# XikunLiu-huskit/GLIO

Hardware: NVIDIA B200
Metric: sliding-window FGO iterations/sec (20 KF, 100k surf pts/scan) (higher is better)
Workload: dtype f64

## Files before the change

### glio_b200/api.py

```python
import ctypes as C
import os

import numpy as np

_HERE = os.path.dirname(os.path.abspath(__file__))
_LIB_PATH = os.path.join(_HERE, "libglio_b200.so")
_LIB = None

HOST, DEVICE = 0, 1
MATCH_VALID, MATCH_FAIL_RADIUS, MATCH_FAIL_PLANE, MATCH_FAIL_WEIGHT = 0, 1, 2, 3


class GlioError(RuntimeError):
    pass


class Params(C.Structure):
    _fields_ = [("kd_max_radius", C.c_double), ("surf_dist_thres", C.c_double), ("lidar_const", C.c_double),
                ("weight_min", C.c_double), ("huber_delta", C.c_double), ("q_lb", C.c_double * 4),
                ("t_lb", C.c_double * 3), ("batch_max_radius", C.c_double), ("batch_dist_thres", C.c_double),
                ("batch_score", C.c_double), ("cell_size", C.c_float), ("keep_debug", C.c_int32), ("unit_score", C.c_int32)]


def lib():
    global _LIB
    if _LIB is None:
        if not os.path.exists(_LIB_PATH):
            raise GlioError(f"{_LIB_PATH} not found: build it with `python -c 'import __graft_entry__ as g; g.build()'` "
                            "(glio_b200 has no CPU fallback)")
        L = C.CDLL(_LIB_PATH)
        L.glio_last_error.restype = C.c_char_p
        L.glio_last_error.argtypes = [C.c_void_p]
        L.glio_stream.restype = C.c_void_p
        L.glio_stream.argtypes = [C.c_void_p]
        L.glio_launch_count.restype = C.c_int64
        L.glio_launch_count.argtypes = [C.c_void_p]
        L.glio_destroy.argtypes = [C.c_void_p]
        L.glio_destroy.restype = None
        L.glio_marg_prior_destroy.argtypes = [C.c_void_p]
        L.glio_marg_prior_destroy.restype = None
        L.glio_marg_prior_create.restype = C.c_void_p
        _LIB = L
    return _LIB


def default_params(**kw):
    p = Params()
    lib().glio_default_params(C.byref(p))
    for k, v in kw.items():
        if k in ("q_lb", "t_lb"):
            arr = getattr(p, k)
            for i, x in enumerate(v):
                arr[i] = float(x)
        else:
            setattr(p, k, v)
    return p


def _ptr(a):
    if a is None:
        return None
    if isinstance(a, np.ndarray):
        return a.ctypes.data_as(C.c_void_p)
    if isinstance(a, int):
        return C.c_void_p(a)
    raise TypeError(type(a))


def _points_arg(xyz):
    if isinstance(xyz, np.ndarray):
        a = np.ascontiguousarray(xyz, dtype=np.float32)
        if a.ndim == 1:
            a = a.reshape(-1, 3)
        return a, _ptr(a), a.shape[0], a.shape[1], HOST
    if hasattr(xyz, "data_ptr"):
        assert xyz.is_cuda and xyz.is_contiguous() and xyz.dtype.itemsize == 4
        return xyz, C.c_void_p(xyz.data_ptr()), xyz.shape[0], xyz.shape[1], DEVICE
    raise TypeError("points must be a numpy array or a CUDA torch tensor")


class Context:
    def __init__(self, device=0, params=None, **kw):
        self._lib = lib()
        self.params = params if params is not None else default_params(**kw)
        self._h = C.c_void_p()
        rc = self._lib.glio_create(C.c_int(device), C.byref(self.params), C.byref(self._h))
        if rc != 0:
            msg = self._lib.glio_last_error(None)
            raise GlioError(f"glio_create failed ({rc}): {msg.decode() if msg else ''}")
        self._keep = []

    def close(self):
        if getattr(self, "_h", None):
            self._lib.glio_destroy(self._h)
            self._h = None

    def __del__(self):
        try:
            self.close()
        except Exception:
            pass

    def _chk(self, rc):
        if rc != 0:
            msg = self._lib.glio_last_error(self._h)
            raise GlioError(f"glio error {rc}: {msg.decode() if msg else ''}")

    @property
    def stream(self):
        return self._lib.glio_stream(self._h)

    @property
    def launch_count(self):
        return int(self._lib.glio_launch_count(self._h))

    def synchronize(self):
        self._chk(self._lib.glio_synchronize(self._h))

    def lidar_pose(self, pose_body):
        pb = np.ascontiguousarray(pose_body, np.float64)
        t2 = np.zeros(3); q2 = np.zeros(4)
        self._lib.glio_lidar_pose(C.byref(self.params), _ptr(pb), _ptr(t2), _ptr(q2))
        return t2, q2

    KERNELS = ["k_feat_curvature", "k_feat_select", "k_feat_voxel", "k_feat_offsets", "k_feat_gather", "k_knn_tile", "k_knn_tile2", "k_defer_scatter", "k_knn_box_start", "k_knn_grow", "k_knn_box_far", "k_knn_far", "k_knn_box_cells", "k_knn_team", "k_make_pairs", "k_knn_search", "k_knn_deferred", "k_knn_thread", "k_knn_box", "k_plane_fit", "k_plane_fit_pair", "k_eval_unary", "k_eval_unary_cost", "k_transform_hist", "k_order_scatter",
               "k_compact", "k_flags", "k_cell_hist", "k_cell_scatter", "k_load_bounds", "k_scan_block", "k_scan_add",
               "k_eval_binary", "k_eval_binary_cost", "k_bin_assemble",
               "k_lm_transform", "k_vox_hist", "k_vox_scatter", "k_vox_sort", "k_vox_flags", "k_vox_centroid", "k_init_bounds"]

    def lib_profile(self, on):
        self._chk(self._lib.glio_profile_enable(self._h, C.c_int(1 if on else 0)))

    def lib_profile_read(self):
        out = {}
        for k in self.KERNELS:
            ms = C.c_double(0); n = C.c_int64(0)
            self._chk(self._lib.glio_profile_get(self._h, k.encode(), C.byref(ms), C.byref(n)))
            if n.value:
                out[k] = (ms.value, int(n.value))
        return out

    def knn_fallback_queries(self, reset=False):
        n = C.c_int64(0)
        self._chk(self._lib.glio_get_stats(self._h, C.byref(n), C.c_int(1 if reset else 0)))
        return int(n.value)

    def get_match_counts(self, W, active=True):
        nm = np.zeros(W, np.int64); na = np.zeros(W, np.int64)
        self._chk(self._lib.glio_get_match_counts(self._h, C.c_int(W), _ptr(nm), _ptr(na)))
        return na if active else nm

    def set_map(self, xyz):
        keep, p, n, stride, mem = _points_arg(xyz)
        self._map_keep = keep
        self._chk(self._lib.glio_set_map(self._h, p, C.c_int64(n), C.c_int(stride), C.c_int(mem)))

    def map_prefetch(self, xyz):
        keep, p, n, stride, mem = _points_arg(xyz)
        assert mem == HOST
        self._map_pf_keep = keep
        self._chk(self._lib.glio_map_prefetch(self._h, p, C.c_int64(n), C.c_int(stride)))

    def localmap_clear(self):
        self._chk(self._lib.glio_localmap_clear(self._h))

    def localmap_push(self, cloud_xyz, t, q, at_front=False):
        keep, p, n, stride, mem = _points_arg(cloud_xyz)
        t = np.ascontiguousarray(t, np.float64); q = np.ascontiguousarray(q, np.float64)
        self._chk(self._lib.glio_localmap_push(self._h, C.c_int(1 if at_front else 0), p, C.c_int64(n), C.c_int(stride), C.c_int(mem), _ptr(t), _ptr(q)))

    def localmap_pop_front(self):
        self._chk(self._lib.glio_localmap_pop_front(self._h))

    def localmap_size(self):
        nf = C.c_int(0); npnt = C.c_int64(0)
        self._chk(self._lib.glio_localmap_size(self._h, C.byref(nf), C.byref(npnt)))
        return nf.value, int(npnt.value)

    def localmap_build(self, leaf=0.4):
        n = C.c_int64(0)
        self._chk(self._lib.glio_localmap_build(self._h, C.c_float(leaf), C.byref(n)))
        return int(n.value)

    def get_map(self):
        n = C.c_int64(0)
        self._chk(self._lib.glio_get_map(self._h, C.c_int64(0), None, C.byref(n)))
        out = np.empty((int(n.value), 3), np.float32)
        self._chk(self._lib.glio_get_map(self._h, C.c_int64(len(out)), _ptr(out), C.byref(n)))
        return out

    def assoc_scan_to_map(self, slot, scan_xyz, t, q):
        keep, p, n, stride, mem = _points_arg(scan_xyz)
        self._keep.append(keep); self._keep = self._keep[-64:]
        t = np.ascontiguousarray(t, np.float64); q = np.ascontiguousarray(q, np.float64)
        nm = C.c_int64(0)
        self._chk(self._lib.glio_assoc_scan_to_map(self._h, C.c_int(slot), p, C.c_int64(n), C.c_int(stride), C.c_int(mem),
                                                   _ptr(t), _ptr(q), C.byref(nm)))
        return int(nm.value)

    def window_set_scans(self, scans):
        args = [_points_arg(s) for s in scans]
        self._scan_keep = [a[0] for a in args]
        W = len(args)
        ptrs = (C.c_void_p * W)(*[a[1] for a in args])
        Q = (C.c_int64 * W)(*[a[2] for a in args])
        strides = {a[3] for a in args}; mems = {a[4] for a in args}
        assert len(strides) == 1 and len(mems) == 1
        self._chk(self._lib.glio_window_set_scans(self._h, C.c_int(W), ptrs, Q, C.c_int(strides.pop()), C.c_int(mems.pop())))

    def window_set_scan(self, slot, scan):
        keep, p, n, stride, mem = _points_arg(scan)
        if not hasattr(self, "_slot_keep"):
            self._slot_keep = {}
        self._slot_keep[slot] = keep
        self._chk(self._lib.glio_window_set_scan(self._h, C.c_int(slot), p, C.c_int64(n), C.c_int(stride), C.c_int(mem)))

    def window_slide(self, W):
        self._chk(self._lib.glio_window_slide(self._h, C.c_int(W)))

    def window_associate(self, poses_body):
        pb = np.ascontiguousarray(poses_body, np.float64).reshape(-1, 7)
        W = len(pb)
        nm = np.zeros(W, np.int64)
        self._chk(self._lib.glio_window_associate(self._h, C.c_int(W), _ptr(pb), _ptr(nm)))
        return nm

    def get_matches(self, slot, capacity):
        cp = np.empty((capacity, 3), np.float32); nsd = np.empty((capacity, 4), np.float32)
        w = np.empty(capacity, np.float32); src = np.empty(capacity, np.int32)
        n = C.c_int64(0)
        self._chk(self._lib.glio_get_matches(self._h, C.c_int(slot), C.c_int64(capacity), _ptr(cp), _ptr(nsd), _ptr(w), _ptr(src), C.byref(n)))
        n = int(n.value)
        return dict(cp=cp[:n], nsd=nsd[:n], weight=w[:n], src=src[:n], n=n)

    def get_assoc_debug(self, slot, Q):
        out = dict(status=np.empty(Q, np.uint8), idx5=np.empty((Q, 5), np.int32), sqd5=np.empty((Q, 5), np.float32),
                   pm=np.empty((Q, 3), np.float32), plane=np.empty((Q, 4), np.float64))
        self._chk(self._lib.glio_get_assoc_debug(self._h, C.c_int(slot), C.c_int64(Q), _ptr(out["status"]), _ptr(out["idx5"]),
                                                 _ptr(out["sqd5"]), _ptr(out["pm"]), _ptr(out["plane"])))
        return out

    def select(self, slot, keep):
        if keep is None:
            self._chk(self._lib.glio_select(self._h, C.c_int(slot), None, C.c_int64(-1)))
            return
        k = np.ascontiguousarray(keep, np.int32)
        self._chk(self._lib.glio_select(self._h, C.c_int(slot), _ptr(k), C.c_int64(len(k))))

    def eval_unary(self, poses_body, jac_kind=0, want_jac=True):
        pb = np.ascontiguousarray(poses_body, np.float64).reshape(-1, 7)
        W = len(pb)
        H = np.zeros((W, 6, 6)) if want_jac else None
        g = np.zeros((W, 6)) if want_jac else None
        cost = np.zeros(W)
        self._chk(self._lib.glio_eval_unary(self._h, C.c_int(W), _ptr(pb), C.c_int(jac_kind), _ptr(H), _ptr(g), _ptr(cost)))
        return dict(H=H, g=g, cost=cost)

    def eval_unary_residuals(self, slot, pose_body, capacity, jac_kind=0):
        pb = np.ascontiguousarray(pose_body, np.float64)
        r = np.empty(capacity); J = np.empty((capacity, 6)); n = C.c_int64(0)
        self._chk(self._lib.glio_eval_unary_residuals(self._h, C.c_int(slot), _ptr(pb), C.c_int(jac_kind), C.c_int64(capacity),
                                                      _ptr(r), _ptr(J), C.byref(n)))
        n = int(n.value)
        return r[:n], J[:n]


class SolverOptions(C.Structure):
    _fields_ = [("max_num_iterations", C.c_int32), ("dogleg_type", C.c_int32), ("use_nonmonotonic_steps", C.c_int32),
                ("max_consecutive_nonmonotonic_steps", C.c_int32), ("initial_trust_region_radius", C.c_double),
                ("max_trust_region_radius", C.c_double), ("min_trust_region_radius", C.c_double),
                ("min_relative_decrease", C.c_double), ("min_lm_diagonal", C.c_double), ("max_lm_diagonal", C.c_double),
                ("max_num_consecutive_invalid_steps", C.c_int32), ("jacobi_scaling", C.c_int32),
                ("function_tolerance", C.c_double), ("gradient_tolerance", C.c_double), ("parameter_tolerance", C.c_double),
                ("fuse_candidate_jacobian", C.c_int32), ("trust_region_strategy", C.c_int32)]


class Iteration(C.Structure):
    _fields_ = [("iteration", C.c_int32), ("step_is_valid", C.c_int32), ("step_is_successful", C.c_int32), ("reserved", C.c_int32),
                ("cost", C.c_double), ("cost_change", C.c_double), ("gradient_max_norm", C.c_double), ("gradient_norm", C.c_double),
# ... 340 lines not shown
```

### glio_b200/csrc/assoc.cu

```cuda
#include "common.cuh"
#include "devmath.cuh"
#include "knn_common.cuh"

namespace glio {

__device__ __forceinline__ int find_seg(const SegDesc* __restrict__ segs, int nseg, int64_t g) {
  int lo = 0, hi = nseg - 1;
  while (lo < hi) {
    int mid = (lo + hi + 1) >> 1;
    if (segs[mid].offset <= g) lo = mid; else hi = mid - 1;
  }
  return lo;
}

__global__ void __launch_bounds__(256) k_transform_hist(GridDesc grid, const SegDesc* __restrict__ segs, int nseg,
                                                        int64_t Qt, float4* __restrict__ pm, uint16_t* __restrict__ segid,
                                                        int* __restrict__ cell_count) {
  const int64_t g = (int64_t)blockIdx.x * blockDim.x + threadIdx.x;
  if (g >= Qt) return;
  const int s = find_seg(segs, nseg, g);
  const SegDesc& sd = segs[s];
  const float* src = sd.src + (g - sd.offset) * sd.stride;
  float p[3] = {src[0], src[1], src[2]};
  PoseD P;
  P.t[0] = sd.t[0]; P.t[1] = sd.t[1]; P.t[2] = sd.t[2];
  P.q[0] = sd.q[0]; P.q[1] = sd.q[1]; P.q[2] = sd.q[2]; P.q[3] = sd.q[3];
  transform_point_f(P, p, p);
  pm[g] = make_float4(p[0], p[1], p[2], 0.f);
  segid[g] = (uint16_t)s;
  atomicAdd(&cell_count[cell_of_clamped(grid, p[0], p[1], p[2])], 1);
}

__global__ void __launch_bounds__(256) k_order_scatter(GridDesc grid, int64_t Qt, const float4* __restrict__ pm,
                                                       const int* __restrict__ cell_start, int* __restrict__ fill,
                                                       float4* __restrict__ pmq) {
  const int64_t g = (int64_t)blockIdx.x * blockDim.x + threadIdx.x;
  if (g >= Qt) return;
  const float4 p = pm[g];
  const int c = cell_of_clamped(grid, p.x, p.y, p.z);
  const int pos = cell_start[c] + atomicAdd(&fill[c], 1);
  pmq[pos] = make_float4(p.x, p.y, p.z, __int_as_float((int)g));
}

constexpr int KNN_WARPS = 4;
constexpr int KNN_SPAN_MAX = 12;

__global__ void __launch_bounds__(32 * KNN_WARPS) k_knn_search(SearchArgs a) {
  __shared__ __align__(16) float sx[KNN_WARPS][32], sy[KNN_WARPS][32], sz[KNN_WARPS][32];
  __shared__ __align__(16) int si[KNN_WARPS][32];
  const int lane = threadIdx.x & 31, wid = threadIdx.x >> 5;
  const int64_t p = ((int64_t)blockIdx.x * KNN_WARPS + wid) * 32 + lane;
  const bool active = p < a.Qt;
  const GridDesc& G = a.grid;
  const float INF = __int_as_float(0x7f800000);
  float qx = 0.f, qy = 0.f, qz = 0.f;
  if (active) { const float4 q4 = a.pmq[p]; qx = q4.x; qy = q4.y; qz = q4.z; }
  const int cx = cell_coord(qx, G.ox, G.inv_cell), cy = cell_coord(qy, G.oy, G.inv_cell), cz = cell_coord(qz, G.oz, G.inv_cell);
  Top5 t;
  top5_init(t);
  const f32x2_t qx2 = pack2(qx, qx), qy2 = pack2(qy, qy), qz2 = pack2(qz, qz);
  const int rmax = (int)ceilf((sqrtf(a.gate_sq) + 2e-3f) * G.inv_cell) + 1;
  const bool far_out = cx < -rmax || cy < -rmax || cz < -rmax || cx >= G.nx + rmax || cy >= G.ny + rmax || cz >= G.nz + rmax;
  bool done = !active || far_out;
  const int* __restrict__ cs = G.cell_start;
  unsigned long long extra_rings = 0;
  for (;;) {
    const unsigned pending = __ballot_sync(0xffffffffu, !done);
    if (!pending) break;
    const int leader = __ffs(pending) - 1;
    const int lcx = __shfl_sync(0xffffffffu, cx, leader), lcy = __shfl_sync(0xffffffffu, cy, leader), lcz = __shfl_sync(0xffffffffu, cz, leader);
    const bool part = !done && cy == lcy && cz == lcz && cx >= lcx && cx < lcx + KNN_SPAN_MAX;
    const int hix = __reduce_max_sync(0xffffffffu, part ? cx : lcx);
    bool unproven = part;
    bool defer = false;
    const int rlim = min(rmax, a.tile_rings);
    for (int r = 1; r <= rlim; ++r) {
      const int xa = lcx - r, xb = hix + r;
      const int x0 = max(xa, 0), x1 = min(xb, G.nx - 1);
      const int z0 = max(lcz - r, 0), z1 = min(lcz + r, G.nz - 1);
      const int y0 = max(lcy - r, 0), y1 = min(lcy + r, G.ny - 1);
      const int nzr = z1 - z0 + 1, nyr = y1 - y0 + 1;
      for (int ri = 0; ri < nzr * nyr; ++ri) {
        {
          int zz = z0 + ri / nyr, yy = y0 + ri % nyr;
          if (r == 1 && lcz >= z0 && lcz <= z1 && lcy >= y0 && lcy <= y1) {
            const int own = (lcz - z0) * nyr + (lcy - y0);
            const int rj = ri == 0 ? own : (ri <= own ? ri - 1 : ri);
            zz = z0 + rj / nyr; yy = y0 + rj % nyr;
          }
          const int z = zz, y = yy;
          const bool zshell = (z == lcz - r) || (z == lcz + r);
          const int row = (z * G.ny + y) * G.nx;
          const bool shell = r == 1 || zshell || (y == lcy - r) || (y == lcy + r);
          for (int part_i = 0; part_i < 2; ++part_i) {
            int s, e;
            if (shell) { if (part_i == 1 || x0 > x1) break; s = __ldg(&cs[row + x0]); e = __ldg(&cs[row + x1 + 1]); }
            else {
              const int xc = part_i == 0 ? xa : xb;
              if (xc < 0 || xc >= G.nx) continue;
              s = __ldg(&cs[row + xc]); e = __ldg(&cs[row + xc + 1]);
            }
            for (int base = s; base < e; base += 32) {
              const int k = base + lane;
              float4 pt = make_float4(1.0e18f, 1.0e18f, 1.0e18f, 0.f);
              if (k < e) pt = __ldg(&G.pts[k]);
              sx[wid][lane] = pt.x; sy[wid][lane] = pt.y; sz[wid][lane] = pt.z; si[wid][lane] = __float_as_int(pt.w);
              __syncwarp();
              const int cnt = min(32, e - base);
              if (unproven) {
                const f32x2_t* px2 = reinterpret_cast<const f32x2_t*>(sx[wid]);
                const f32x2_t* py2 = reinterpret_cast<const f32x2_t*>(sy[wid]);
                const f32x2_t* pz2 = reinterpret_cast<const f32x2_t*>(sz[wid]);
                for (int j = 0; j < cnt; j += 2) {
                  const f32x2_t dx = sub2(qx2, px2[j >> 1]), dy = sub2(qy2, py2[j >> 1]), dz = sub2(qz2, pz2[j >> 1]);
                  const f32x2_t a2 = fma2(dz, dz, fma2(dy, dy, mul2(dx, dx)));
                  float a0, a1; unpack2(a2, a0, a1);
                  const float thr = key_dist(t.k4) * 1.000001f;
                  if (a0 <= thr) top5_push(t, l2_simple(qx, qy, qz, sx[wid][j], sy[wid][j], sz[wid][j]), si[wid][j]);
                  if (j + 1 < cnt && a1 <= key_dist(t.k4) * 1.000001f) top5_push(t, l2_simple(qx, qy, qz, sx[wid][j + 1], sy[wid][j + 1], sz[wid][j + 1]), si[wid][j + 1]);
                }
              }
              __syncwarp();
            }
          }
        }
      }
      if (unproven) {
        float b = INF;
        if (xa > 0)               b = fminf(b, qx - (G.ox + (float)xa * G.cell));
        if (xb < G.nx - 1)        b = fminf(b, (G.ox + (float)(xb + 1) * G.cell) - qx);
        if (lcy - r > 0)          b = fminf(b, qy - (G.oy + (float)(lcy - r) * G.cell));
        if (lcy + r < G.ny - 1)   b = fminf(b, (G.oy + (float)(lcy + r + 1) * G.cell) - qy);
        if (lcz - r > 0)          b = fminf(b, qz - (G.oz + (float)(lcz - r) * G.cell));
        if (lcz + r < G.nz - 1)   b = fminf(b, (G.oz + (float)(lcz + r + 1) * G.cell) - qz);
        const float bs = b * 0.999f - 2e-3f;
        if ((b == INF) || (bs > 0.f && key_dist(t.k4) <= bs * bs)) unproven = false;
        else if (r == rlim && rlim < rmax) defer = true;
      }
      if (!__ballot_sync(0xffffffffu, unproven)) break;
    }
    if (part) done = true;
    const unsigned dm = __ballot_sync(0xffffffffu, defer);
    if (dm) {
      unsigned int base = 0;
      if (lane == 0) { base = atomicAdd(a.n_deferred, (unsigned int)__popc(dm)); extra_rings += __popc(dm); }
      base = __shfl_sync(0xffffffffu, base, 0);
      if (defer) a.deferred[base + __popc(dm & ((1u << lane) - 1u))] = (uint32_t)p;
    }
  }
  if (a.n_fallback && lane == 0 && extra_rings) atomicAdd(a.n_fallback, extra_rings);
  if (active) {
    a.knn_idx[0 * a.Qt + p] = key_idx(t.k0); a.knn_idx[1 * a.Qt + p] = key_idx(t.k1); a.knn_idx[2 * a.Qt + p] = key_idx(t.k2);
    a.knn_idx[3 * a.Qt + p] = key_idx(t.k3); a.knn_idx[4 * a.Qt + p] = key_idx(t.k4);
    a.knn_sqd[0 * a.Qt + p] = key_dist(t.k0); a.knn_sqd[1 * a.Qt + p] = key_dist(t.k1); a.knn_sqd[2 * a.Qt + p] = key_dist(t.k2);
    a.knn_sqd[3 * a.Qt + p] = key_dist(t.k3); a.knn_sqd[4 * a.Qt + p] = key_dist(t.k4);
  }
}

__global__ void __launch_bounds__(128, 7) k_knn_thread(SearchArgs a) {
  __shared__ int sbnd[18 * 128];
  const int64_t p = (int64_t)blockIdx.x * blockDim.x + threadIdx.x;
  if (p >= a.Qt) return;
  const GridDesc& g = a.grid;
  const float4 q4 = a.pmq[p];
  const float qx = q4.x, qy = q4.y, qz = q4.z;
  Top5 t; top5_init(t);
  const int cx = cell_coord(qx, g.ox, g.inv_cell), cy = cell_coord(qy, g.oy, g.inv_cell), cz = cell_coord(qz, g.oz, g.inv_cell);
  const int rmax = (int)ceilf((sqrtf(a.gate_sq) + 2e-3f) * g.inv_cell) + 1;
  const bool far_out = cx < -rmax || cy < -rmax || cz < -rmax || cx >= g.nx + rmax || cy >= g.ny + rmax || cz >= g.nz + rmax;
  float d4f = __int_as_float(0x7f800000);
  if (!far_out) thread_rings(g, qx, qy, qz, cx, cy, cz, 1, rmax, rmax, t, d4f, sbnd + threadIdx.x);
  store_top5(a, p, t);
}

template <bool START_OWN>
__global__ void __launch_bounds__(128, 6) k_knn_box(SearchArgs a) {
  __shared__ int sbnd[18 * 128];
  const int64_t p = (int64_t)blockIdx.x * blockDim.x + threadIdx.x;
  if (p >= a.Qt) return;
  const GridDesc& g = a.grid;
  const float4 q4 = a.pmq[p];
  const float qx = q4.x, qy = q4.y, qz = q4.z;
  Top5 t; top5_init(t);
  const int cx = cell_coord(qx, g.ox, g.inv_cell), cy = cell_coord(qy, g.oy, g.inv_cell), cz = cell_coord(qz, g.oz, g.inv_cell);
  const float gate_r = sqrtf(a.gate_sq) + 2e-3f;
  const int rmax = (int)ceilf(gate_r * g.inv_cell) + 1;
  const bool far_out = cx < -rmax || cy < -rmax || cz < -rmax || cx >= g.nx + rmax || cy >= g.ny + rmax || cz >= g.nz + rmax;
  float d4f = __int_as_float(0x7f800000);
  if (!far_out) {
    int lx, hx, ly, hy, lz, hz;
    if (START_OWN) {
      lx = hx = cx; ly = hy = cy; lz = hz = cz;
      scan_rows(g, cx, cx, cy, cy, cz, cz, qx, qy, qz, t, d4f);
// ... 71 lines not shown
    }
    if (lane == 0) {
      a.knn_idx[0 * a.Qt + p] = key_idx(t.k0); a.knn_idx[1 * a.Qt + p] = key_idx(t.k1); a.knn_idx[2 * a.Qt + p] = key_idx(t.k2);
      a.knn_idx[3 * a.Qt + p] = key_idx(t.k3); a.knn_idx[4 * a.Qt + p] = key_idx(t.k4);
      a.knn_sqd[0 * a.Qt + p] = key_dist(t.k0); a.knn_sqd[1 * a.Qt + p] = key_dist(t.k1); a.knn_sqd[2 * a.Qt + p] = key_dist(t.k2);
      a.knn_sqd[3 * a.Qt + p] = key_dist(t.k3); a.knn_sqd[4 * a.Qt + p] = key_dist(t.k4);
    }
  }
}

struct FitArgs {
  int64_t Qt;
  const float4* pm;
  const float4* pmq;
  const int32_t* knn_idx;
  const float* knn_sqd;
  AssocGates gates;
  const float4* pts_sorted;
  const int* sorted_pos;
  const float* oth_local;
  int oth_stride;
  uint8_t* status;
  float4* nsd;
  float* weight;
  double* normal_cent;
  int32_t* idx5;
  float* sqd5;
  double* plane;
};

#ifndef GLIO_FIT_REGATHER
#define GLIO_FIT_REGATHER 1
#endif
#ifndef GLIO_FIT_MINBLOCKS
#define GLIO_FIT_MINBLOCKS (GLIO_FIT_REGATHER ? 5 : 4)
#endif
template <bool PAIR>
__global__ void __launch_bounds__(128, GLIO_FIT_MINBLOCKS) k_plane_fit(FitArgs a) {
  const int64_t p = (int64_t)blockIdx.x * blockDim.x + threadIdx.x;
  if (p >= a.Qt) return;
  const float4 q4 = a.pmq[p];
  const int64_t g = __float_as_int(q4.w);
  int id[5];
#pragma unroll
  for (int j = 0; j < 5; ++j) id[j] = a.knn_idx[(int64_t)j * a.Qt + p];
  const float d4 = a.knn_sqd[4 * a.Qt + p];
  uint8_t st;
  float w = 0.f;
  double n[3] = {0, 0, 0}, d = 0;
  double nl[3] = {0, 0, 0}, cl[3] = {0, 0, 0};
  if (id[4] != 0x7fffffff && (double)d4 < a.gates.max_radius) {
#if GLIO_FIT_REGATHER
    int pos[5];
#pragma unroll
    for (int j = 0; j < 5; ++j) pos[j] = __ldg(&a.sorted_pos[id[j]]);
    double Aw[3][5];
#pragma unroll
    for (int j = 0; j < 5; ++j) {
      const float4 m = __ldg(&a.pts_sorted[pos[j]]);
      Aw[0][j] = (double)m.x; Aw[1][j] = (double)m.y; Aw[2][j] = (double)m.z;
    }
    double x[3];
    plane_solve5(Aw, x);
    plane_from_solution(x, n, d);
    bool ok = true;
#pragma unroll
    for (int j = 0; j < 5; ++j) {
      const float4 m = __ldg(&a.pts_sorted[pos[j]]);
      const double v = dadd(dadd(dadd(dmul(n[0], (double)m.x), dmul(n[1], (double)m.y)), dmul(n[2], (double)m.z)), d);
      if (fabs(v) > a.gates.dist_thres) ok = false;
    }
#else
    double A[3][5];
#pragma unroll
    for (int j = 0; j < 5; ++j) {
      const float4 m = __ldg(&a.pts_sorted[__ldg(&a.sorted_pos[id[j]])]);
      A[0][j] = (double)m.x; A[1][j] = (double)m.y; A[2][j] = (double)m.z;
    }
    double Aw[3][5];
#pragma unroll
    for (int c = 0; c < 3; ++c)
#pragma unroll
      for (int j = 0; j < 5; ++j) Aw[c][j] = A[c][j];
    double x[3];
    plane_solve5(Aw, x);
    plane_from_solution(x, n, d);
    bool ok = true;
#pragma unroll
    for (int j = 0; j < 5; ++j) {
      const double v = dadd(dadd(dadd(dmul(n[0], A[0][j]), dmul(n[1], A[1][j])), dmul(n[2], A[2][j])), d);
      if (fabs(v) > a.gates.dist_thres) ok = false;
    }
#endif
    if (ok) {
      w = weight_of(n, d, q4.x, q4.y, q4.z);
      st = ((double)w > a.gates.weight_min) ? GLIO_MATCH_VALID : GLIO_MATCH_FAIL_WEIGHT;
    } else st = GLIO_MATCH_FAIL_PLANE;
    if (PAIR && st == GLIO_MATCH_VALID) {
      double Al[3][5];
      double sx = 0.0, sy = 0.0, sz = 0.0;
#pragma unroll
      for (int j = 0; j < 5; ++j) {
        const float* lp = a.oth_local + (int64_t)id[j] * a.oth_stride;
        Al[0][j] = (double)lp[0]; Al[1][j] = (double)lp[1]; Al[2][j] = (double)lp[2];
        sx = dadd(sx, Al[0][j]); sy = dadd(sy, Al[1][j]); sz = dadd(sz, Al[2][j]);
      }
      cl[0] = sx / 5.0; cl[1] = sy / 5.0; cl[2] = sz / 5.0;
      double xl[3], dl;
      plane_solve5(Al, xl);
      plane_from_solution(xl, nl, dl);
    }
  } else st = GLIO_MATCH_FAIL_RADIUS;

  a.status[g] = st;
  if (!PAIR) {
    float4 o = make_float4(0.f, 0.f, 0.f, 0.f);
    if (st == GLIO_MATCH_VALID) {
      o.x = (float)dmul((double)w, n[0]); o.y = (float)dmul((double)w, n[1]);
      o.z = (float)dmul((double)w, n[2]); o.w = (float)dmul((double)w, d);
    }
    a.nsd[g] = o;
  } else {
    double* nc = a.normal_cent + 6 * g;
    const bool v = st == GLIO_MATCH_VALID;
    nc[0] = v ? nl[0] : 0.0; nc[1] = v ? nl[1] : 0.0; nc[2] = v ? nl[2] : 0.0;
    nc[3] = v ? cl[0] : 0.0; nc[4] = v ? cl[1] : 0.0; nc[5] = v ? cl[2] : 0.0;
  }
  a.weight[g] = (st == GLIO_MATCH_VALID || st == GLIO_MATCH_FAIL_WEIGHT) ? w : 0.f;
  if (a.idx5) {
#pragma unroll
    for (int j = 0; j < 5; ++j) {
      a.idx5[5 * g + j] = (id[j] == 0x7fffffff) ? -1 : id[j];
      a.sqd5[5 * g + j] = a.knn_sqd[(int64_t)j * a.Qt + p];
    }
    a.plane[4 * g] = n[0]; a.plane[4 * g + 1] = n[1]; a.plane[4 * g + 2] = n[2]; a.plane[4 * g + 3] = d;
  }
}

void assoc_run(const GridBuild& gb, const SegDesc* d_segs, int nseg, const AssocWork& w, const AssocGates& gates,
               const float* oth_local, int oth_stride, DevBuf<int>& cell_count, DevBuf<int>& cell_pos,
               DevBuf<int>& scan_tmp, cudaStream_t st, LaunchCounter& lc) {
  const GridDesc& grid = gb.desc;
  const int64_t Qt = w.Qt;
  if (Qt <= 0) return;
  GLIO_REQUIRE(Qt < ((int64_t)1 << 31), GLIO_ERR_ARG, "assoc_run: too many queries in one launch");
  GLIO_REQUIRE(nseg > 0 && nseg < 65536, GLIO_ERR_ARG, "assoc_run: bad segment count");
  const int64_t ncell = (int64_t)grid.nx * grid.ny * grid.nz;
  cell_count.reserve((size_t)ncell + 2);
  cell_pos.reserve((size_t)ncell + 2);
  GLIO_CUDA_TRY(cudaMemsetAsync(cell_count.p, 0, (size_t)(ncell + 1) * sizeof(int), st));
  const unsigned nb = (unsigned)((Qt + 255) / 256);
  lc.begin("k_transform_hist", st); k_transform_hist<<<nb, 256, 0, st>>>(grid, d_segs, nseg, Qt, w.pm, w.seg, cell_count.p); lc.end(st);
  exclusive_scan_i32(cell_count.p, cell_pos.p, ncell + 1, scan_tmp, st, lc);
  GLIO_CUDA_TRY(cudaMemsetAsync(cell_count.p, 0, (size_t)(ncell + 1) * sizeof(int), st));
  lc.begin("k_order_scatter", st); k_order_scatter<<<nb, 256, 0, st>>>(grid, Qt, w.pm, cell_pos.p, cell_count.p, w.pmq); lc.end(st);
  SearchArgs sa;
  sa.grid = grid; sa.Qt = Qt; sa.pm = w.pm; sa.pmq = w.pmq; sa.gate_sq = (float)gates.max_radius;
  sa.knn_idx = w.knn_idx; sa.knn_sqd = w.knn_sqd; sa.n_fallback = w.n_fallback; sa.store_all_sqd = w.idx5 != nullptr;
  sa.tile_rings = w.tile_rings; sa.grow_mode = w.grow_mode; sa.deferred = w.deferred; sa.n_deferred = w.n_deferred;
  GLIO_CUDA_TRY(cudaMemsetAsync(w.n_deferred, 0, sizeof(unsigned int), st));
  const unsigned ns = (unsigned)((Qt + 32 * KNN_WARPS - 1) / (32 * KNN_WARPS));
  if (w.knn_mode == 7) {
    knn_box_cells_run(sa, st, lc);
  } else if (w.knn_mode == 6) {
    knn_box_far_run(sa, st, lc);
  } else if (w.knn_mode == 5) {
    knn_box2_run(sa, cell_count, scan_tmp, st, lc);
  } else if (w.knn_mode == 4) {
    knn_tile_run(sa, gb.pairs.p, cell_count, scan_tmp, st, lc);
  } else if (w.knn_mode == 2 || w.knn_mode == 3) {
    lc.begin("k_knn_box", st);
    if (w.knn_mode == 3) k_knn_box<true><<<(unsigned)((Qt + 127) / 128), 128, 0, st>>>(sa);
    else k_knn_box<false><<<(unsigned)((Qt + 127) / 128), 128, 0, st>>>(sa);
    lc.end(st);
  } else if (w.knn_mode == 1) {
    lc.begin("k_knn_thread", st); k_knn_thread<<<(unsigned)((Qt + 127) / 128), 128, 0, st>>>(sa); lc.end(st);
  } else {
    lc.begin("k_knn_search", st); k_knn_search<<<ns, 32 * KNN_WARPS, 0, st>>>(sa); lc.end(st);
    if (w.tile_rings < 32) { lc.begin("k_knn_deferred", st); k_knn_deferred<<<148 * 8, 128, 0, st>>>(sa); lc.end(st); }
  }
  FitArgs fa;
  fa.Qt = Qt; fa.pm = w.pm; fa.pmq = w.pmq; fa.knn_idx = w.knn_idx; fa.knn_sqd = w.knn_sqd; fa.gates = gates;
  fa.pts_sorted = gb.pts.p; fa.sorted_pos = gb.sorted_pos.p; fa.oth_local = oth_local; fa.oth_stride = oth_stride;
  fa.status = w.status; fa.nsd = w.nsd; fa.weight = w.weight; fa.normal_cent = w.normal_cent;
  fa.idx5 = w.idx5; fa.sqd5 = w.sqd5; fa.plane = w.plane;
  const unsigned nk = (unsigned)((Qt + 127) / 128);
  lc.begin(w.normal_cent ? "k_plane_fit_pair" : "k_plane_fit", st);
  if (w.normal_cent) k_plane_fit<true><<<nk, 128, 0, st>>>(fa);
  else k_plane_fit<false><<<nk, 128, 0, st>>>(fa);
  lc.end(st);
  GLIO_CUDA_TRY(cudaGetLastError());
}

__global__ void __launch_bounds__(256) k_flags(const uint8_t* __restrict__ status, int64_t Qt, int* __restrict__ flags) {
  const int64_t g = (int64_t)blockIdx.x * blockDim.x + threadIdx.x;
  if (g < Qt) flags[g] = status[g] == GLIO_MATCH_VALID ? 1 : 0;
  if (g == Qt) flags[g] = 0;
}

__global__ void __launch_bounds__(256) k_compact(const SegDesc* __restrict__ segs, int64_t Qt, const uint16_t* __restrict__ segid,
                                                 const uint8_t* __restrict__ status, const int* __restrict__ pos,
                                                 const float4* __restrict__ nsd, const float* __restrict__ weight,
                                                 const double* __restrict__ normal_cent, const CompactDst* __restrict__ dst) {
  const int64_t g = (int64_t)blockIdx.x * blockDim.x + threadIdx.x;
  if (g >= Qt) return;
  if (status[g] != GLIO_MATCH_VALID) return;
  const int s = segid[g];
  const SegDesc& sd = segs[s];
  const int lp = pos[g] - pos[sd.offset];
  const int64_t li = g - sd.offset;
  const float* src = sd.src + li * sd.stride;
  const CompactDst d = dst[s];
  d.cpw[lp] = make_float4(src[0], src[1], src[2], weight[g]);
  if (d.nsd) d.nsd[lp] = nsd[g];
  if (d.nc) {
#pragma unroll
    for (int k = 0; k < 6; ++k) d.nc[6 * (int64_t)lp + k] = normal_cent[6 * g + k];
  }
  d.src[lp] = (int32_t)li;
}

__global__ void k_seg_counts(const SegDesc* __restrict__ segs, int nseg, const int* __restrict__ pos, int* __restrict__ counts) {
  const int s = blockIdx.x * blockDim.x + threadIdx.x;
  if (s < nseg) counts[s] = pos[segs[s].offset + segs[s].count] - pos[segs[s].offset];
}

void compact_count(const AssocWork& w, const SegDesc* d_segs, int nseg, int* d_flags, int* d_pos, DevBuf<int>& scan_tmp,
                   int* d_counts, cudaStream_t st, LaunchCounter& lc) {
  const int64_t Qt = w.Qt;
  const unsigned nb = (unsigned)((Qt + 1 + 255) / 256);
  lc.begin("k_flags", st); k_flags<<<nb, 256, 0, st>>>(w.status, Qt, d_flags); lc.end(st);
  exclusive_scan_i32(d_flags, d_pos, Qt + 1, scan_tmp, st, lc);
  lc.begin("k_seg_counts", st); k_seg_counts<<<(nseg + 127) / 128, 128, 0, st>>>(d_segs, nseg, d_pos, d_counts); lc.end(st);
  GLIO_CUDA_TRY(cudaGetLastError());
}

void compact_scatter(const AssocWork& w, const SegDesc* d_segs, int nseg, const int* d_pos, const void* d_dst, cudaStream_t st,
                     LaunchCounter& lc) {
  const int64_t Qt = w.Qt;
  const unsigned nb = (unsigned)((Qt + 255) / 256);
  lc.begin("k_compact", st); k_compact<<<nb, 256, 0, st>>>(d_segs, Qt, w.seg, w.status, d_pos, w.nsd, w.weight, w.normal_cent, (const CompactDst*)d_dst); lc.end(st);
  GLIO_CUDA_TRY(cudaGetLastError());
}

void compact_run(const AssocWork& w, const SegDesc* d_segs, int nseg, int* d_flags, int* d_pos, DevBuf<int>& scan_tmp,
                 const void* d_dst , int* d_counts, cudaStream_t st, LaunchCounter& lc) {
  compact_count(w, d_segs, nseg, d_flags, d_pos, scan_tmp, d_counts, st, lc);
  compact_scatter(w, d_segs, nseg, d_pos, d_dst, st, lc);
}

__global__ void __launch_bounds__(256) k_gather_sel(const int32_t* __restrict__ keep, int64_t n, int64_t n_match,
                                                    const float4* __restrict__ cpw, const float4* __restrict__ nsd,
                                                    const double* __restrict__ nc, float4* __restrict__ o_cpw,
                                                    float4* __restrict__ o_nsd, double* __restrict__ o_nc, int* __restrict__ bad) {
  const int64_t i = (int64_t)blockIdx.x * blockDim.x + threadIdx.x;
  if (i >= n) return;
  const int k = keep[i];
  if (k < 0 || k >= n_match) { atomicAdd(bad, 1); return; }
  o_cpw[i] = cpw[k];
  if (nsd) o_nsd[i] = nsd[k];
  if (nc) {
#pragma unroll
    for (int c = 0; c < 6; ++c) o_nc[6 * i + c] = nc[6 * (int64_t)k + c];
  }
}

void gather_selection(const int32_t* d_keep, int64_t n, int64_t n_match, const float4* cpw, const float4* nsd, const double* nc,
                      float4* o_cpw, float4* o_nsd, double* o_nc, int* d_bad, cudaStream_t st, LaunchCounter& lc) {
  if (n <= 0) return;
  lc.begin("k_gather_sel", st); k_gather_sel<<<(unsigned)((n + 255) / 256), 256, 0, st>>>(d_keep, n, n_match, cpw, nsd, nc, o_cpw, o_nsd, o_nc, d_bad); lc.end(st);
  GLIO_CUDA_TRY(cudaGetLastError());
}

}
```

### glio_b200/csrc/grid.cu

```cuda
#include "common.cuh"
#include "devmath.cuh"

namespace glio {

static std::string g_err;
void set_global_error(const std::string& m) { g_err = m; }
const char* global_error() { return g_err.c_str(); }

constexpr int SCAN_T = 1024;
constexpr int SCAN_IPT = 4;
constexpr int SCAN_B = SCAN_T * SCAN_IPT;

__global__ void __launch_bounds__(SCAN_T) k_scan_block(const int* __restrict__ in, int* __restrict__ out,
                                                        int* __restrict__ block_sums, int64_t n) {
  __shared__ int warp_sums[32];
  const int64_t base = (int64_t)blockIdx.x * SCAN_B + (int64_t)threadIdx.x * SCAN_IPT;
  int v[SCAN_IPT];
  int tsum = 0;
#pragma unroll
  for (int k = 0; k < SCAN_IPT; ++k) {
    v[k] = (base + k < n) ? in[base + k] : 0;
    tsum += v[k];
  }
  int x = tsum;
  const int lane = threadIdx.x & 31, wid = threadIdx.x >> 5;
#pragma unroll
  for (int o = 1; o < 32; o <<= 1) {
    int y = __shfl_up_sync(0xffffffffu, x, o);
    if (lane >= o) x += y;
  }
  if (lane == 31) warp_sums[wid] = x;
  __syncthreads();
  if (wid == 0) {
    int w = warp_sums[lane];
#pragma unroll
    for (int o = 1; o < 32; o <<= 1) {
      int y = __shfl_up_sync(0xffffffffu, w, o);
      if (lane >= o) w += y;
    }
    warp_sums[lane] = w;
  }
  __syncthreads();
  int excl = x - tsum + (wid > 0 ? warp_sums[wid - 1] : 0);
#pragma unroll
  for (int k = 0; k < SCAN_IPT; ++k) {
    if (base + k < n) out[base + k] = excl;
    excl += v[k];
  }
  if (threadIdx.x == SCAN_T - 1 && block_sums) block_sums[blockIdx.x] = excl;
}

__global__ void __launch_bounds__(SCAN_T) k_scan_add(int* __restrict__ out, const int* __restrict__ block_offs, int64_t n) {
  const int add = block_offs[blockIdx.x];
  const int64_t base = (int64_t)blockIdx.x * SCAN_B + (int64_t)threadIdx.x * SCAN_IPT;
#pragma unroll
  for (int k = 0; k < SCAN_IPT; ++k)
    if (base + k < n) out[base + k] += add;
}

__global__ void __launch_bounds__(SCAN_T) k_scan_add2(int* __restrict__ out, const int* __restrict__ block_sums, int64_t n) {
  __shared__ int warp_sums[32];
  int part = 0;
  for (int i = threadIdx.x; i < (int)blockIdx.x; i += SCAN_T) part += block_sums[i];
#pragma unroll
  for (int o = 16; o > 0; o >>= 1) part += __shfl_xor_sync(0xffffffffu, part, o);
  if ((threadIdx.x & 31) == 0) warp_sums[threadIdx.x >> 5] = part;
  __syncthreads();
  int add = 0;
#pragma unroll
  for (int w = 0; w < SCAN_T / 32; ++w) add += warp_sums[w];
  if (blockIdx.x == 0) return;
  const int64_t base = (int64_t)blockIdx.x * SCAN_B + (int64_t)threadIdx.x * SCAN_IPT;
#pragma unroll
  for (int k = 0; k < SCAN_IPT; ++k)
    if (base + k < n) out[base + k] += add;
}

static void scan_rec(const int* in, int* out, int64_t n, int* tmp, int64_t tmp_cap, cudaStream_t st, LaunchCounter& lc) {
  const int64_t nb = (n + SCAN_B - 1) / SCAN_B;
  if (nb <= 1) {
    lc.begin("k_scan_block", st); k_scan_block<<<1, SCAN_T, 0, st>>>(in, out, nullptr, n); lc.end(st);
    return;
  }
  GLIO_REQUIRE(nb <= tmp_cap, GLIO_ERR_STATE, "scan scratch too small");
  lc.begin("k_scan_block", st); k_scan_block<<<(unsigned)nb, SCAN_T, 0, st>>>(in, out, tmp, n); lc.end(st);
  if (nb <= 4096) {
    lc.begin("k_scan_add", st); k_scan_add2<<<(unsigned)nb, SCAN_T, 0, st>>>(out, tmp, n); lc.end(st);
    return;
  }
  scan_rec(tmp, tmp, nb, tmp + nb, tmp_cap - nb, st, lc);
  lc.begin("k_scan_add", st); k_scan_add<<<(unsigned)nb, SCAN_T, 0, st>>>(out, tmp, n); lc.end(st);
}

void exclusive_scan_i32(const int* in, int* out, int64_t n, DevBuf<int>& tmp, cudaStream_t st, LaunchCounter& lc) {
  if (n <= 0) return;
  int64_t need = 0;
  for (int64_t m = (n + SCAN_B - 1) / SCAN_B; m > 1; m = (m + SCAN_B - 1) / SCAN_B) need += m;
  need += 8;
  tmp.reserve((size_t)need);
  scan_rec(in, out, n, tmp.p, (int64_t)tmp.cap, st, lc);
  GLIO_CUDA_TRY(cudaGetLastError());
}

__device__ __forceinline__ int float_to_ordered(float f) {
  int i = __float_as_int(f);
  return i ^ ((i >> 31) & 0x7fffffff);
}
__host__ __device__ __forceinline__ float ordered_to_float_h(int i) {
  int j = i ^ ((i >> 31) & 0x7fffffff);
#ifdef __CUDA_ARCH__
  return __int_as_float(j);
#else
  float f; memcpy(&f, &j, 4); return f;
#endif
}

__global__ void __launch_bounds__(256) k_load_bounds(const float* __restrict__ xyz, int stride, int64_t n, PoseD pose, int has_pose,
                                                     float4* __restrict__ out, int* __restrict__ bounds ) {
  float mn[3] = {3.0e38f, 3.0e38f, 3.0e38f}, mx[3] = {-3.0e38f, -3.0e38f, -3.0e38f};
  for (int64_t i = (int64_t)blockIdx.x * blockDim.x + threadIdx.x; i < n; i += (int64_t)gridDim.x * blockDim.x) {
    float p[3] = {xyz[i * stride], xyz[i * stride + 1], xyz[i * stride + 2]};
    if (has_pose) transform_point_f(pose, p, p);
    out[i] = make_float4(p[0], p[1], p[2], __int_as_float((int)i));
#pragma unroll
    for (int d = 0; d < 3; ++d) { mn[d] = fminf(mn[d], p[d]); mx[d] = fmaxf(mx[d], p[d]); }
  }
#pragma unroll
  for (int d = 0; d < 3; ++d) {
#pragma unroll
    for (int o = 16; o > 0; o >>= 1) {
      mn[d] = fminf(mn[d], __shfl_xor_sync(0xffffffffu, mn[d], o));
      mx[d] = fmaxf(mx[d], __shfl_xor_sync(0xffffffffu, mx[d], o));
    }
  }
  __shared__ float smn[8][3], smx[8][3];
  const int wid = threadIdx.x >> 5;
  if ((threadIdx.x & 31) == 0) {
#pragma unroll
    for (int d = 0; d < 3; ++d) { smn[wid][d] = mn[d]; smx[wid][d] = mx[d]; }
  }
  __syncthreads();
  if (threadIdx.x < 3) {
    const int d = threadIdx.x;
    float a = smn[0][d], b = smx[0][d];
    for (int w = 1; w < (int)(blockDim.x >> 5); ++w) { a = fminf(a, smn[w][d]); b = fmaxf(b, smx[w][d]); }
    atomicMin(&bounds[d], float_to_ordered(a));
    atomicMax(&bounds[3 + d], float_to_ordered(b));
  }
}

__global__ void k_init_bounds(int* bounds) {
  if (threadIdx.x < 3) bounds[threadIdx.x] = 0x7fffffff;
  else if (threadIdx.x < 6) bounds[threadIdx.x] = (int)0x80000000;
}

__global__ void __launch_bounds__(256) k_cell_hist(const float4* __restrict__ pts, int64_t n, GridDesc g, int* __restrict__ count) {
  for (int64_t i = (int64_t)blockIdx.x * blockDim.x + threadIdx.x; i < n; i += (int64_t)gridDim.x * blockDim.x) {
    float4 p = pts[i];
    atomicAdd(&count[cell_of_clamped(g, p.x, p.y, p.z)], 1);
  }
}

__global__ void __launch_bounds__(256) k_cell_scatter(const float4* __restrict__ pts, int64_t n, GridDesc g,
                                                      const int* __restrict__ cell_start, int* __restrict__ fill,
                                                      float4* __restrict__ sorted, int* __restrict__ sorted_pos) {
  for (int64_t i = (int64_t)blockIdx.x * blockDim.x + threadIdx.x; i < n; i += (int64_t)gridDim.x * blockDim.x) {
    float4 p = pts[i];
    int c = cell_of_clamped(g, p.x, p.y, p.z);
    int pos = cell_start[c] + atomicAdd(&fill[c], 1);
    sorted[pos] = p;
    sorted_pos[i] = pos;
  }
}

__global__ void __launch_bounds__(256) k_make_pairs(const float4* __restrict__ sorted, int64_t n, PairRec* __restrict__ pairs) {
  const int64_t np = (n + 1) >> 1;
  for (int64_t k = (int64_t)blockIdx.x * blockDim.x + threadIdx.x; k < np; k += (int64_t)gridDim.x * blockDim.x) {
    const float4 a = sorted[2 * k];
    float4 b = make_float4(PAIR_FAR, 0.f, 0.f, __int_as_float(0x7fffffff));
    if (2 * k + 1 < n) b = sorted[2 * k + 1];
    PairRec r;
    r.x0 = a.x; r.x1 = b.x; r.y0 = a.y; r.y1 = b.y; r.z0 = a.z; r.z1 = b.z; r.i0 = __float_as_int(a.w); r.i1 = __float_as_int(b.w);
    pairs[k] = r;
  }
}

void grid_build(GridBuild& gb, const float* d_xyz, int stride, int64_t n, const double* t, const double* q,
                float cell_size_hint, float pts_per_cell, cudaStream_t st, LaunchCounter& lc) {
  GLIO_REQUIRE(n > 0 && n < (int64_t)1 << 31, GLIO_ERR_ARG, "grid_build: point count out of range");
  gb.tmp4.reserve((size_t)n);
  gb.pts.reserve((size_t)n);
  gb.sorted_pos.reserve((size_t)n);
  gb.bounds.reserve(8);
  PoseD pose{};
  int has_pose = 0;
  if (t && q) { has_pose = 1; for (int k = 0; k < 3; ++k) pose.t[k] = t[k]; for (int k = 0; k < 4; ++k) pose.q[k] = q[k]; }
  int* d_bounds = (int*)gb.bounds.p;
  lc.begin("k_init_bounds", st); k_init_bounds<<<1, 32, 0, st>>>(d_bounds); lc.end(st);
  const int nb = (int)std::min<int64_t>((n + 255) / 256, 148 * 8);
  lc.begin("k_load_bounds", st); k_load_bounds<<<nb, 256, 0, st>>>(d_xyz, stride, n, pose, has_pose, gb.tmp4.p, d_bounds); lc.end(st);
  int hb[6];
  GLIO_CUDA_TRY(cudaMemcpyAsync(hb, d_bounds, sizeof(hb), cudaMemcpyDeviceToHost, st));
  GLIO_CUDA_TRY(cudaStreamSynchronize(st));
  float mn[3], mx[3];
  for (int d = 0; d < 3; ++d) { mn[d] = ordered_to_float_h(hb[d]); mx[d] = ordered_to_float_h(hb[3 + d]); }
  for (int d = 0; d < 3; ++d)
    GLIO_REQUIRE(std::isfinite(mn[d]) && std::isfinite(mx[d]), GLIO_ERR_ARG, "grid_build: non-finite point coordinates");
  float L[3] = {mx[0] - mn[0] + 1e-3f, mx[1] - mn[1] + 1e-3f, mx[2] - mn[2] + 1e-3f};
  float cell = cell_size_hint;
  if (!(cell > 0)) {
    double area = 2.0 * ((double)L[0] * L[1] + (double)L[1] * L[2] + (double)L[0] * L[2]);
    cell = (float)std::sqrt(pts_per_cell * area / (double)n);
    if (cell < 0.05f) cell = 0.05f;
    if (cell > 4.0f) cell = 4.0f;
  }
  const double max_cells = 48.0e6;
  for (;;) {
    double nc = std::ceil(L[0] / cell + 1) * std::ceil(L[1] / cell + 1) * std::ceil(L[2] / cell + 1);
    if (nc <= max_cells) break;
    cell *= 1.26f;
  }
  GridDesc& g = gb.desc;
  g.cell = cell; g.inv_cell = 1.0f / cell;
  g.ox = mn[0] - 0.5f * cell; g.oy = mn[1] - 0.5f * cell; g.oz = mn[2] - 0.5f * cell;
  g.nx = (int)std::floor((mx[0] - g.ox) / cell) + 2;
  g.ny = (int)std::floor((mx[1] - g.oy) / cell) + 2;
  g.nz = (int)std::floor((mx[2] - g.oz) / cell) + 2;
  g.npts = n;
  const int64_t ncell = (int64_t)g.nx * g.ny * g.nz;
  gb.cell_start.reserve((size_t)ncell + 2);
  gb.fill.reserve((size_t)ncell + 2);
  GLIO_CUDA_TRY(cudaMemsetAsync(gb.fill.p, 0, (size_t)(ncell + 1) * sizeof(int), st));
  lc.begin("k_cell_hist", st); k_cell_hist<<<nb, 256, 0, st>>>(gb.tmp4.p, n, g, gb.fill.p); lc.end(st);
  exclusive_scan_i32(gb.fill.p, gb.cell_start.p, ncell + 1, gb.scan_tmp, st, lc);
  GLIO_CUDA_TRY(cudaMemsetAsync(gb.fill.p, 0, (size_t)(ncell + 1) * sizeof(int), st));
  lc.begin("k_cell_scatter", st); k_cell_scatter<<<nb, 256, 0, st>>>(gb.tmp4.p, n, g, gb.cell_start.p, gb.fill.p, gb.pts.p, gb.sorted_pos.p); lc.end(st);
  if (gb.build_pairs) {
    gb.pairs.reserve((size_t)((n + 1) / 2 + 1));
    lc.begin("k_make_pairs", st); k_make_pairs<<<nb, 256, 0, st>>>(gb.pts.p, n, gb.pairs.p); lc.end(st);
  }
  GLIO_CUDA_TRY(cudaGetLastError());
  g.cell_start = gb.cell_start.p;
  g.pts = gb.pts.p;
}

__global__ void __launch_bounds__(256) k_lm_transform(const float* __restrict__ xyz, int stride, int64_t n, PoseD pose, float4* __restrict__ out) {
  for (int64_t i = (int64_t)blockIdx.x * blockDim.x + threadIdx.x; i < n; i += (int64_t)gridDim.x * blockDim.x) {
    float p[3] = {xyz[i * stride], xyz[i * stride + 1], xyz[i * stride + 2]};
    transform_point_f(pose, p, p);
    out[i] = make_float4(p[0], p[1], p[2], 0.f);
  }
}

// ... 163 lines not shown
```

Measured before the change: 2141.

## Replace multi-kernel exclusive scan with single-pass decoupled look-back scan

The recursive block-scan plus add-kernel scheme becomes one kernel. It takes tile ids from an atomic ticket and resolves cross-tile prefixes through per-tile aggregate/inclusive status words read with relaxed loads, so scan launches drop from two or more to one plus a memset. Separately, the order-scatter kernel now uses the scanned cell offsets directly as atomic cursors, which removes a second memset of the cell-count array. The trade-offs are spin-waiting on predecessor tiles, and cell_pos being overwritten with cell end offsets after the scatter.

```diff
diff --git a/glio_b200/api.py b/glio_b200/api.py
--- a/glio_b200/api.py
+++ b/glio_b200/api.py
@@ -124,7 +124,7 @@
         return t2, q2
 
     KERNELS = ["k_feat_curvature", "k_feat_select", "k_feat_voxel", "k_feat_offsets", "k_feat_gather", "k_knn_tile", "k_knn_tile2", "k_defer_scatter", "k_knn_box_start", "k_knn_grow", "k_knn_box_far", "k_knn_far", "k_knn_box_cells", "k_knn_team", "k_make_pairs", "k_knn_search", "k_knn_deferred", "k_knn_thread", "k_knn_box", "k_plane_fit", "k_plane_fit_pair", "k_eval_unary", "k_eval_unary_cost", "k_transform_hist", "k_order_scatter",
-               "k_compact", "k_flags", "k_cell_hist", "k_cell_scatter", "k_load_bounds", "k_scan_block", "k_scan_add",
+               "k_compact", "k_flags", "k_cell_hist", "k_cell_scatter", "k_load_bounds", "k_scan",
                "k_eval_binary", "k_eval_binary_cost", "k_bin_assemble",
                "k_lm_transform", "k_vox_hist", "k_vox_scatter", "k_vox_sort", "k_vox_flags", "k_vox_centroid", "k_init_bounds"]
 
diff --git a/glio_b200/csrc/assoc.cu b/glio_b200/csrc/assoc.cu
--- a/glio_b200/csrc/assoc.cu
+++ b/glio_b200/csrc/assoc.cu
@@ -32,13 +32,12 @@
 }
 
 __global__ void __launch_bounds__(256) k_order_scatter(GridDesc grid, int64_t Qt, const float4* __restrict__ pm,
-                                                       const int* __restrict__ cell_start, int* __restrict__ fill,
-                                                       float4* __restrict__ pmq) {
+                                                       int* __restrict__ cell_cursor, float4* __restrict__ pmq) {
   const int64_t g = (int64_t)blockIdx.x * blockDim.x + threadIdx.x;
   if (g >= Qt) return;
   const float4 p = pm[g];
   const int c = cell_of_clamped(grid, p.x, p.y, p.z);
-  const int pos = cell_start[c] + atomicAdd(&fill[c], 1);
+  const int pos = atomicAdd(&cell_cursor[c], 1);
   pmq[pos] = make_float4(p.x, p.y, p.z, __int_as_float((int)g));
 }
 
@@ -416,8 +415,7 @@
   const unsigned nb = (unsigned)((Qt + 255) / 256);
   lc.begin("k_transform_hist", st); k_transform_hist<<<nb, 256, 0, st>>>(grid, d_segs, nseg, Qt, w.pm, w.seg, cell_count.p); lc.end(st);
   exclusive_scan_i32(cell_count.p, cell_pos.p, ncell + 1, scan_tmp, st, lc);
-  GLIO_CUDA_TRY(cudaMemsetAsync(cell_count.p, 0, (size_t)(ncell + 1) * sizeof(int), st));
-  lc.begin("k_order_scatter", st); k_order_scatter<<<nb, 256, 0, st>>>(grid, Qt, w.pm, cell_pos.p, cell_count.p, w.pmq); lc.end(st);
+  lc.begin("k_order_scatter", st); k_order_scatter<<<nb, 256, 0, st>>>(grid, Qt, w.pm, cell_pos.p, w.pmq); lc.end(st);
   SearchArgs sa;
   sa.grid = grid; sa.Qt = Qt; sa.pm = w.pm; sa.pmq = w.pmq; sa.gate_sq = (float)gates.max_radius;
   sa.knn_idx = w.knn_idx; sa.knn_sqd = w.knn_sqd; sa.n_fallback = w.n_fallback; sa.store_all_sqd = w.idx5 != nullptr;
diff --git a/glio_b200/csrc/grid.cu b/glio_b200/csrc/grid.cu
--- a/glio_b200/csrc/grid.cu
+++ b/glio_b200/csrc/grid.cu
@@ -11,10 +11,24 @@
 constexpr int SCAN_IPT = 4;
 constexpr int SCAN_B = SCAN_T * SCAN_IPT;
 
-__global__ void __launch_bounds__(SCAN_T) k_scan_block(const int* __restrict__ in, int* __restrict__ out,
-                                                        int* __restrict__ block_sums, int64_t n) {
+__device__ __forceinline__ unsigned long long ld_state(const unsigned long long* p) {
+  unsigned long long v;
+  asm volatile("ld.relaxed.gpu.global.u64 %0, [%1];" : "=l"(v) : "l"(p) : "memory");
+  return v;
+}
+__device__ __forceinline__ void st_state(unsigned long long* p, unsigned long long v) {
+  asm volatile("st.relaxed.gpu.global.u64 [%0], %1;" ::"l"(p), "l"(v) : "memory");
+}
+constexpr unsigned long long SCAN_AGG = 1ull << 32, SCAN_INC = 2ull << 32;
+
+__global__ void __launch_bounds__(SCAN_T) k_scan_onepass(const int* __restrict__ in, int* __restrict__ out, int64_t n,
+                                                         unsigned long long* __restrict__ state, unsigned int* __restrict__ ticket) {
   __shared__ int warp_sums[32];
-  const int64_t base = (int64_t)blockIdx.x * SCAN_B + (int64_t)threadIdx.x * SCAN_IPT;
+  __shared__ int s_tile, s_prefix;
+  if (threadIdx.x == 0) s_tile = (int)atomicAdd(ticket, 1u);
+  __syncthreads();
+  const int tile = s_tile;
+  const int64_t base = (int64_t)tile * SCAN_B + (int64_t)threadIdx.x * SCAN_IPT;
   int v[SCAN_IPT];
   int tsum = 0;
 #pragma unroll
@@ -39,66 +53,48 @@
       if (lane >= o) w += y;
     }
     warp_sums[lane] = w;
+    const int total = __shfl_sync(0xffffffffu, w, 31);
+    int prefix = 0;
+    if (tile == 0) {
+      if (lane == 0) st_state(&state[0], SCAN_INC | (unsigned int)total);
+    } else {
+      if (lane == 0) st_state(&state[tile], SCAN_AGG | (unsigned int)total);
+      int j = tile - 1;
+      for (;;) {
+        const int idx = j - lane;
+        unsigned long long s = idx >= 0 ? ld_state(&state[idx]) : SCAN_INC;
+        if (__any_sync(0xffffffffu, (s >> 32) == 0)) { __nanosleep(20); continue; }
+        const unsigned inc = __ballot_sync(0xffffffffu, (s >> 32) == 2);
+        const int stop = inc ? __ffs(inc) - 1 : 31;
+        int c = lane <= stop ? (int)(unsigned int)s : 0;
+#pragma unroll
+        for (int o = 16; o > 0; o >>= 1) c += __shfl_xor_sync(0xffffffffu, c, o);
+        prefix += c;
+        if (inc) break;
+        j -= 32;
+      }
+      if (lane == 0) st_state(&state[tile], SCAN_INC | (unsigned int)(prefix + total));
+    }
+    if (lane == 0) s_prefix = prefix;
   }
   __syncthreads();
-  int excl = x - tsum + (wid > 0 ? warp_sums[wid - 1] : 0);
+  int excl = x - tsum + (wid > 0 ? warp_sums[wid - 1] : 0) + s_prefix;
 #pragma unroll
   for (int k = 0; k < SCAN_IPT; ++k) {
     if (base + k < n) out[base + k] = excl;
     excl += v[k];
   }
-  if (threadIdx.x == SCAN_T - 1 && block_sums) block_sums[blockIdx.x] = excl;
-}
-
-__global__ void __launch_bounds__(SCAN_T) k_scan_add(int* __restrict__ out, const int* __restrict__ block_offs, int64_t n) {
-  const int add = block_offs[blockIdx.x];
-  const int64_t base = (int64_t)blockIdx.x * SCAN_B + (int64_t)threadIdx.x * SCAN_IPT;
-#pragma unroll
-  for (int k = 0; k < SCAN_IPT; ++k)
-    if (base + k < n) out[base + k] += add;
-}
-
-__global__ void __launch_bounds__(SCAN_T) k_scan_add2(int* __restrict__ out, const int* __restrict__ block_sums, int64_t n) {
-  __shared__ int warp_sums[32];
-  int part = 0;
-  for (int i = threadIdx.x; i < (int)blockIdx.x; i += SCAN_T) part += block_sums[i];
-#pragma unroll
-  for (int o = 16; o > 0; o >>= 1) part += __shfl_xor_sync(0xffffffffu, part, o);
-  if ((threadIdx.x & 31) == 0) warp_sums[threadIdx.x >> 5] = part;
-  __syncthreads();
-  int add = 0;
-#pragma unroll
-  for (int w = 0; w < SCAN_T / 32; ++w) add += warp_sums[w];
-  if (blockIdx.x == 0) return;
-  const int64_t base = (int64_t)blockIdx.x * SCAN_B + (int64_t)threadIdx.x * SCAN_IPT;
-#pragma unroll
-  for (int k = 0; k < SCAN_IPT; ++k)
-    if (base + k < n) out[base + k] += add;
-}
-
-static void scan_rec(const int* in, int* out, int64_t n, int* tmp, int64_t tmp_cap, cudaStream_t st, LaunchCounter& lc) {
-  const int64_t nb = (n + SCAN_B - 1) / SCAN_B;
-  if (nb <= 1) {
-    lc.begin("k_scan_block", st); k_scan_block<<<1, SCAN_T, 0, st>>>(in, out, nullptr, n); lc.end(st);
-    return;
-  }
-  GLIO_REQUIRE(nb <= tmp_cap, GLIO_ERR_STATE, "scan scratch too small");
-  lc.begin("k_scan_block", st); k_scan_block<<<(unsigned)nb, SCAN_T, 0, st>>>(in, out, tmp, n); lc.end(st);
-  if (nb <= 4096) {
-    lc.begin("k_scan_add", st); k_scan_add2<<<(unsigned)nb, SCAN_T, 0, st>>>(out, tmp, n); lc.end(st);
-    return;
-  }
-  scan_rec(tmp, tmp, nb, tmp + nb, tmp_cap - nb, st, lc);
-  lc.begin("k_scan_add", st); k_scan_add<<<(unsigned)nb, SCAN_T, 0, st>>>(out, tmp, n); lc.end(st);
 }
 
 void exclusive_scan_i32(const int* in, int* out, int64_t n, DevBuf<int>& tmp, cudaStream_t st, LaunchCounter& lc) {
   if (n <= 0) return;
-  int64_t need = 0;
-  for (int64_t m = (n + SCAN_B - 1) / SCAN_B; m > 1; m = (m + SCAN_B - 1) / SCAN_B) need += m;
-  need += 8;
-  tmp.reserve((size_t)need);
-  scan_rec(in, out, n, tmp.p, (int64_t)tmp.cap, st, lc);
+  const int64_t nt = (n + SCAN_B - 1) / SCAN_B;
+  GLIO_REQUIRE(nt < ((int64_t)1 << 31), GLIO_ERR_ARG, "exclusive_scan_i32: too many items");
+  tmp.reserve((size_t)(2 * nt + 2));
+  unsigned long long* state = reinterpret_cast<unsigned long long*>(tmp.p);
+  unsigned int* ticket = reinterpret_cast<unsigned int*>(tmp.p + 2 * nt);
+  GLIO_CUDA_TRY(cudaMemsetAsync(tmp.p, 0, (size_t)(2 * nt + 1) * sizeof(int), st));
+  lc.begin("k_scan", st); k_scan_onepass<<<(unsigned)nt, SCAN_T, 0, st>>>(in, out, n, state, ticket); lc.end(st);
   GLIO_CUDA_TRY(cudaGetLastError());
 }
 
```

New measurement: 2135 (median of 6 runs). No clear change (-0.3%).
